# lijun9250lj/video-steganography-PCAMV

Measured on AMD Instinct MI355X. Metric: 1080p macroblocks/s (embed on), higher is better.
Workload: dtype u8

## Files before the change

### video-steganography-pcamv_amd/csrc/pcamv_prims_gpu.h

```cpp
#ifndef PCAMV_PRIMS_GPU_H
#define PCAMV_PRIMS_GPU_H
#include "pcamv_common.h"

__device__ __forceinline__ int pcamv_lane_id(void) { int l = (int)(threadIdx.x & 63); asm volatile("" : "+v"(l)); return l; }
#ifndef PCAMV_RD_LO
#define PCAMV_RD_LO 0
#endif
#define LANE() (PCAMV_RD_LO ? (int)(threadIdx.x & 63) : pcamv_lane_id())
__device__ __forceinline__ uint32_t clamp_u8(int v)
{
    asm volatile("" : "+v"(v));
    return (uint32_t)(v < 0 ? 0 : v > 255 ? 255 : v);
}
__device__ __forceinline__ uint32_t ld4u(const uint8_t *p) { uint32_t v; __builtin_memcpy(&v, p, 4); return v; }
__device__ __forceinline__ uint32_t lds4(const uint8_t *p) { return *(const uint32_t *)p; }
__device__ __forceinline__ void sts4(uint8_t *p, uint32_t v) { *(uint32_t *)p = v; }
__device__ __forceinline__ uint32_t avg4(uint32_t a, uint32_t b) { return __builtin_amdgcn_lerp(a, b, 0x01010101u); }
__device__ __forceinline__ int dpp_qp1(int v) { return __builtin_amdgcn_update_dpp(0, v, 0xB1, 0xf, 0xf, false); }
__device__ __forceinline__ int dpp_qp2(int v) { return __builtin_amdgcn_update_dpp(0, v, 0x4E, 0xf, 0xf, false); }
__device__ __forceinline__ int dpp_hmir(int v) { return __builtin_amdgcn_update_dpp(0, v, 0x141, 0xf, 0xf, false); }
__device__ __forceinline__ int dpp_mir(int v) { return __builtin_amdgcn_update_dpp(0, v, 0x140, 0xf, 0xf, false); }

__device__ __forceinline__ int group_sum(int v, int g)
{
    if (g >= 2) v += dpp_qp1(v);
    if (g >= 4) v += dpp_qp2(v);
    if (g >= 8) v += dpp_hmir(v);
    if (g >= 16) v += dpp_mir(v);
    return v;
}
__device__ __forceinline__ int wave_sum_all(int v)
{
    v = group_sum(v, 16);
    return __builtin_amdgcn_readlane(v, 0) + __builtin_amdgcn_readlane(v, 16) + __builtin_amdgcn_readlane(v, 32) + __builtin_amdgcn_readlane(v, 48);
}

__device__ __forceinline__ int hadamard4x4_abs(const uint32_t e[4], const uint32_t r[4])
{
    int t[4][4], s = 0;
#pragma unroll
    for (int y = 0; y < 4; y++) {
        int d0 = (int)(e[y] & 255) - (int)(r[y] & 255), d1 = (int)((e[y] >> 8) & 255) - (int)((r[y] >> 8) & 255);
        int d2 = (int)((e[y] >> 16) & 255) - (int)((r[y] >> 16) & 255), d3 = (int)(e[y] >> 24) - (int)(r[y] >> 24);
        int s01 = d0 + d1, d01 = d0 - d1, s23 = d2 + d3, d23 = d2 - d3;
        t[y][0] = s01 + s23; t[y][1] = d01 + d23; t[y][2] = s01 - s23; t[y][3] = d01 - d23;
    }
#pragma unroll
    for (int x = 0; x < 4; x++) {
        int s01 = t[0][x] + t[1][x], d01 = t[0][x] - t[1][x], s23 = t[2][x] + t[3][x], d23 = t[2][x] - t[3][x];
        s += iabs(s01 + s23) + iabs(d01 + d23) + iabs(s01 - s23) + iabs(d01 - d23);
    }
    return s;
}

__device__ __forceinline__ uint32_t chroma_row4(const FrameDev &F, int plane, int cx, int cy, int mvx, int mvy)
{
    int dx = mvx & 7, dy = mvy & 7;
    int cA = (8 - dx) * (8 - dy), cB = dx * (8 - dy), cC = (8 - dx) * dy, cD = dx * dy;
    const uint8_t *s = (plane ? F.chroma[1] : F.chroma[0]) + (ptrdiff_t)(cy + (mvy >> 3)) * F.cstride + cx + (mvx >> 3);
    uint32_t a0 = ld4u(s), a1 = s[4], b0 = ld4u(s + F.cstride), b1 = s[F.cstride + 4];
    uint32_t o = 0;
#pragma unroll
    for (int i = 0; i < 4; i++) {
        int p00 = (a0 >> (8 * i)) & 255, p01 = i < 3 ? (a0 >> (8 * i + 8)) & 255 : a1;
        int p10 = (b0 >> (8 * i)) & 255, p11 = i < 3 ? (b0 >> (8 * i + 8)) & 255 : b1;
        o |= (uint32_t)((cA * p00 + cB * p01 + cC * p10 + cD * p11 + 32) >> 6) << (8 * i);
    }
    return o;
}


__device__ __forceinline__ int rfl(int v) { return __builtin_amdgcn_readfirstlane(v); }
__device__ __forceinline__ int wave_min_i32(int v)
{
    v = imin(v, dpp_qp1(v)); v = imin(v, dpp_qp2(v)); v = imin(v, dpp_hmir(v)); v = imin(v, dpp_mir(v));
    return imin(imin(__builtin_amdgcn_readlane(v, 0), __builtin_amdgcn_readlane(v, 16)),
                imin(__builtin_amdgcn_readlane(v, 32), __builtin_amdgcn_readlane(v, 48)));
}

typedef const __attribute__((address_space(1))) uint8_t *gp8;
typedef const __attribute__((address_space(1))) int16_t *gp16;
typedef uint32_t __attribute__((aligned(1))) u32u;
typedef uint64_t __attribute__((aligned(1))) u64u;
typedef short v2s __attribute__((ext_vector_type(2)));
__device__ __forceinline__ uint32_t gld4(gp8 base, uint32_t off) { return *(const __attribute__((address_space(1))) u32u *)(base + off); }
__device__ __forceinline__ uint64_t gld8(gp8 base, uint32_t off) { return *(const __attribute__((address_space(1))) u64u *)(base + off); }
__device__ __forceinline__ int gld_cost(gp8 tab, uint32_t i) { return (int)*(const __attribute__((address_space(1))) int16_t *)(tab + (i << 1)); }
__device__ __forceinline__ int prim_mv_cost(const FrameDev &F, int d)
{
    const int i = rfl(d) + PCAMV_COST_MV_CENTRE;
    const __attribute__((address_space(4))) uint32_t *t = (const __attribute__((address_space(4))) uint32_t *)(F.cost_mv - PCAMV_COST_MV_CENTRE);
    const uint32_t w = t[i >> 1];
    return (int)(int16_t)(w >> (16 * (i & 1)));
}
__device__ __forceinline__ uint32_t mul24u(uint32_t a, uint32_t b) { return __umul24(a, b); }
__device__ __forceinline__ int mul24s(int a, int b) { return __mul24(a, b); }
__device__ __forceinline__ int mad24s(int a, int b, int c) { return __mul24(a, b) + c; }
__device__ __forceinline__ uint32_t lsw_x(uint32_t x, uint32_t lskip) { return mul24u(mul24u(x, 18725u) >> 19, lskip) + x; }
__device__ __forceinline__ v2s as_v2s(uint32_t v) { return __builtin_bit_cast(v2s, v); }
__device__ __forceinline__ uint32_t as_u32(v2s v) { return __builtin_bit_cast(uint32_t, v); }

__device__ __forceinline__ void pk_cols(const uint32_t r[4], uint32_t o[8])
{
#pragma unroll
    for (int x = 0; x < 4; x++) {
        const uint32_t sel = 0x0c040c00u + (uint32_t)x * 0x00010001u;
        o[x] = __builtin_amdgcn_perm(r[1], r[0], sel);
        o[4 + x] = __builtin_amdgcn_perm(r[3], r[2], sel);
    }
}
__device__ __forceinline__ int satd4x4_half(const uint32_t ec[8], const uint32_t r[4])
{
    uint32_t rc[8];
    pk_cols(r, rc);
    v2s t[8];
#pragma unroll
    for (int g = 0; g < 2; g++) {
        v2s d0 = as_v2s(ec[4 * g]) - as_v2s(rc[4 * g]), d1 = as_v2s(ec[4 * g + 1]) - as_v2s(rc[4 * g + 1]);
        v2s d2 = as_v2s(ec[4 * g + 2]) - as_v2s(rc[4 * g + 2]), d3 = as_v2s(ec[4 * g + 3]) - as_v2s(rc[4 * g + 3]);
        v2s s01 = d0 + d1, d01 = d0 - d1, s23 = d2 + d3, d23 = d2 - d3;
        t[4 * g] = s01 + s23; t[4 * g + 1] = d01 + d23; t[4 * g + 2] = s01 - s23; t[4 * g + 3] = d01 - d23;
    }
    v2s acc = {0, 0};
    const v2s z = {0, 0};
#pragma unroll
    for (int x = 0; x < 4; x++) {
        v2s S = t[x] + t[4 + x], D = t[x] - t[4 + x];
        v2s aS = __builtin_elementwise_max(S, z - S), aD = __builtin_elementwise_max(D, z - D);
        v2s U = as_v2s(__builtin_amdgcn_perm(as_u32(aD), as_u32(aS), 0x05040100u));
        v2s V = as_v2s(__builtin_amdgcn_perm(as_u32(aD), as_u32(aS), 0x07060302u));
        acc += __builtin_elementwise_max(U, V);
    }
    return (int)acc.x + (int)acc.y;
}

__device__ __forceinline__ void chroma_rows_load(gp8 cb, uint32_t cstride, uint32_t off, uint64_t row[5])
{
#pragma unroll
    for (int k = 0; k < 5; k++) row[k] = gld8(cb + (size_t)k * cstride, off);
}
__device__ __forceinline__ void chroma_block4_rows(const uint64_t row[5], int mvx, int mvy, uint32_t r[4])
{
    const int dx = mvx & 7, dy = mvy & 7;
    const uint32_t W = mul24u(8 - dx, 8 - dy) | mul24u(dx, 8 - dy) << 8 | mul24u(8 - dx, dy) << 16 | mul24u(dx, dy) << 24;
    uint32_t w[5][4];
#pragma unroll
    for (int k = 0; k < 5; k++) {
        const uint32_t lo = (uint32_t)row[k], hi = (uint32_t)(row[k] >> 32);
        w[k][0] = lo; w[k][1] = __builtin_amdgcn_alignbit(hi, lo, 8); w[k][2] = __builtin_amdgcn_alignbit(hi, lo, 16); w[k][3] = __builtin_amdgcn_alignbit(hi, lo, 24);
    }
#pragma unroll
    for (int k = 0; k < 4; k++) {
        uint32_t o = 0;
#pragma unroll
        for (int i = 0; i < 4; i++) {
            const uint32_t px = __builtin_amdgcn_perm(w[k + 1][i], w[k][i], 0x05040100u);
            o |= (__builtin_amdgcn_udot4(px, W, 32u, false) >> 6) << (8 * i);
        }
        r[k] = o;
    }
}
__device__ __forceinline__ void chroma_block4(gp8 cb, uint32_t cstride, uint32_t off, int mvx, int mvy, uint32_t r[4])
{
    uint64_t row[5];
    chroma_rows_load(cb, cstride, off, row);
    chroma_block4_rows(row, mvx, mvy, r);
}

__device__ __forceinline__ uint32_t wld4(const MBLocal *L, int b)
{
    const uint32_t *w = L->win + (b >> 2);
    return __builtin_amdgcn_alignbit(w[1], w[0], (uint32_t)(b & 3) * 8u);
}
__device__ __forceinline__ void prim_win_load(const FrameDev &F, MBLocal *L, int bmx, int bmy)
{
    PCAMV_WAVE_SYNC();
    const int lane = LANE();
    const int x0 = L->mb_x * 16 + PCAMV_PAD + ((bmx - 3) >> 2), y0 = L->mb_y * 16 + PCAMV_PAD + ((bmy - 3) >> 2);
    const int cx0 = L->mb_x * 8 + PCAMV_CPAD + ((bmx - 3) >> 3), cy0 = L->mb_y * 8 + PCAMV_CPAD + ((bmy - 3) >> 3);
    const gp8 lb = (gp8)F.luma_base, cb = (gp8)F.chroma_base[0];
    const uint32_t lskip = (uint32_t)F.lskip, psz = (uint32_t)F.plane_size, cstride = (uint32_t)F.cstride, cps = (uint32_t)F.cplane_size;
    for (int i = lane; i < 4 * WIN_LH * (WIN_LW / 4); i += 64) {
        const int pl = i / (WIN_LH * (WIN_LW / 4)), r = (i / (WIN_LW / 4)) % WIN_LH, c = i % (WIN_LW / 4);
        L->win[i] = gld4(lb, (uint32_t)pl * psz + (uint32_t)(y0 + r) * PCAMV_LROW + lsw_x((uint32_t)(x0 + 4 * c), lskip));
    }
    for (int i = lane; i < 2 * WIN_CH * (WIN_CW / 4); i += 64) {
        const int pl = i / (WIN_CH * (WIN_CW / 4)), r = (i / (WIN_CW / 4)) % WIN_CH, c = i % (WIN_CW / 4);
        L->win[4 * WIN_LP / 4 + i] = gld4(cb, (uint32_t)pl * cps + (uint32_t)(cy0 + r) * cstride + (uint32_t)(cx0 + 4 * c));
    }
    if (lane == 0) { L->win_x0 = x0; L->win_y0 = y0; L->win_cx0 = cx0; L->win_cy0 = cy0; }
    PCAMV_WAVE_SYNC();
}
__device__ __forceinline__ void chroma_block4_win(const MBLocal *L, int b, int mvx, int mvy, uint32_t r[4])
{
    const int dx = mvx & 7, dy = mvy & 7;
    const uint32_t W = mul24u(8 - dx, 8 - dy) | mul24u(dx, 8 - dy) << 8 | mul24u(8 - dx, dy) << 16 | mul24u(dx, dy) << 24;
    const uint32_t sh = (uint32_t)(b & 3) * 8u;
    uint32_t w[5][4];
#pragma unroll
    for (int k = 0; k < 5; k++) {
        const uint32_t *p = L->win + ((b + k * WIN_CW) >> 2);
        const uint32_t lo = __builtin_amdgcn_alignbit(p[1], p[0], sh), hi = __builtin_amdgcn_alignbit(p[2], p[1], sh);
        w[k][0] = lo; w[k][1] = __builtin_amdgcn_alignbit(hi, lo, 8); w[k][2] = __builtin_amdgcn_alignbit(hi, lo, 16); w[k][3] = __builtin_amdgcn_alignbit(hi, lo, 24);
    }
#pragma unroll
    for (int k = 0; k < 4; k++) {
        uint32_t o = 0;
#pragma unroll
        for (int i = 0; i < 4; i++) {
            const uint32_t px = __builtin_amdgcn_perm(w[k + 1][i], w[k][i], 0x05040100u);
            o |= (__builtin_amdgcn_udot4(px, W, 32u, false) >> 6) << (8 * i);
        }
        r[k] = o;
    }
}

struct EvalEnv { const int16_t *cost_mv; const uint8_t *luma_base, *chroma_base; long long plane_size, cplane_size; int lskip, cstride; int *trace; int trace_mb; };
__device__ __forceinline__ EvalRes eval_list_body(const EvalEnv &F, MBLocal *L, const uint8_t *enc, int ip_, int xoff_, int yoff_,
                                                  int n_, int flags_, int mvp0_, int mvp1_)
{
    const int ip = rfl(ip_), xoff = rfl(xoff_), yoff = rfl(yoff_), n = rfl(n_), flags = rfl(flags_), mvp0 = rfl(mvp0_), mvp1 = rfl(mvp1_);
    const int lane = LANE();
    const int lgn = lg_nblk_of(ip), lgw = lg_w4_of(ip), nblk = 1 << lgn;
    const int satd = flags & EV_SATD;
    const gp8 cost_tab = (gp8)(F.cost_mv - PCAMV_COST_MV_CENTRE);
    PCAMV_WAVE_SYNC();
    const unsigned long long t_ev = PROF_T();
    PROF_CNT(32, 1); PROF_CNT(33, n);
    int key_acc = 0x7fffffff;
    {
        const int slot = lane >> lgn, blk = lane & (nblk - 1);
        const int px = xoff + 4 * (blk & ((1 << lgw) - 1)), py = yoff + 4 * (blk >> lgw);
        uint32_t e[4], ec[8];
        const uint8_t *encl = (flags & EV_SRC4) ? enc + (slot & 3) * 384 : enc;
#pragma unroll
        for (int k = 0; k < 4; k++) e[k] = lds4(encl + (py + k) * 16 + px);
        if (satd) pk_cols(e, ec);
        const gp8 lb = (gp8)F.luma_base;
        const uint32_t stride = PCAMV_LROW, psz = (uint32_t)F.plane_size, lskip = (uint32_t)F.lskip;
        const gp8 lb1 = lb + stride, lb2 = lb1 + stride, lb3 = lb2 + stride;
        const uint32_t rowbase = (uint32_t)(L->mb_y * 16 + py + PCAMV_PAD) * stride, colbase = (uint32_t)(L->mb_x * 16 + px + PCAMV_PAD);
        const int cpp = 64 >> lgn;
        for (int p0 = 0; p0 < n; p0 += cpp) {
            const int c = p0 + slot;
            const uint32_t xy = L->cxy[c < n ? c : 0];
            const bool act = c < n && xy != CAND_NONE;
            const int mvx = act ? (int)(int16_t)(xy & 0xffffu) : 0, mvy = act ? (int)(int16_t)(xy >> 16) : 0;
            const uint32_t o = rowbase + (uint32_t)((mvy >> 2) * (int)stride) + lsw_x(colbase + (uint32_t)(mvx >> 2), lskip);
            int mvb0 = 0, mvb1 = 0;
            if (!(flags & EV_NOMV)) { mvb0 = gld_cost(cost_tab, (uint32_t)(mvx - mvp0 + PCAMV_COST_MV_CENTRE)); mvb1 = gld_cost(cost_tab, (uint32_t)(mvy - mvp1 + PCAMV_COST_MV_CENTRE)); }
            uint32_t r[4];
            if (flags & EV_WIN) {
                const int dx = mvx & 3, dy = mvy & 3;
                const int wb = (L->mb_y * 16 + py + PCAMV_PAD + (mvy >> 2) - L->win_y0) * WIN_LW + (L->mb_x * 16 + px + PCAMV_PAD + (mvx >> 2) - L->win_x0);
                const int ba = wb + ((dx != 0) + 2 * (dy == 2)) * WIN_LP + (dy == 3 ? WIN_LW : 0);
#pragma unroll
                for (int k = 0; k < 4; k++) r[k] = wld4(L, ba + k * WIN_LW);
                if ((dx | dy) & 1) {
                    const int bb = wb + (dy ? (2 + (dx == 2)) * WIN_LP : 0) + (dx == 3);
#pragma unroll
                    for (int k = 0; k < 4; k++) r[k] = avg4(r[k], wld4(L, bb + k * WIN_LW));
                }
            } else if (flags & EV_FPEL) {
                r[0] = gld4(lb, o); r[1] = gld4(lb1, o); r[2] = gld4(lb2, o); r[3] = gld4(lb3, o);
            } else {
                const int dx = mvx & 3, dy = mvy & 3;
                const uint32_t oa = o + (dx != 0 ? psz : 0u) + (dy == 2 ? 2u * psz : 0u) + (dy == 3 ? stride : 0u);
                r[0] = gld4(lb, oa); r[1] = gld4(lb1, oa); r[2] = gld4(lb2, oa); r[3] = gld4(lb3, oa);
                if ((dx | dy) & 1) {
                    const uint32_t ob = o + (dy ? (dx == 2 ? 3u * psz : 2u * psz) : 0u) + (dx == 3);
                    r[0] = avg4(r[0], gld4(lb, ob)); r[1] = avg4(r[1], gld4(lb1, ob));
                    r[2] = avg4(r[2], gld4(lb2, ob)); r[3] = avg4(r[3], gld4(lb3, ob));
                }
            }
            asm volatile("" : "+v"(mvb0), "+v"(mvb1), "+v"(r[0]), "+v"(r[1]), "+v"(r[2]), "+v"(r[3]));
            int v;
            if (satd) v = satd4x4_half(ec, r);
            else {
                uint32_t sa = 0;
#pragma unroll
                for (int k = 0; k < 4; k++) sa = __builtin_amdgcn_sad_u8(e[k], r[k], sa);
                v = (int)sa;
            }
            v = group_sum(v, nblk) + mvb0 + mvb1;
            if (blk == 0 && c < n) L->ccost[c] = act ? v : PCAMV_COST_MAX;
            if (blk == 0 && act) key_acc = imin(key_acc, (v << 6) | c);
        }
    }
    PCAMV_WAVE_SYNC();
    if ((flags & EV_CHROMA) && ip <= PIX_8x8) {
        const int lgnb = lgn - 2, nb = 1 << lgnb, lgcw = lgw - 1;
        const int slot = lane >> (lgnb + 1), plane = (lane >> lgnb) & 1, blk = lane & (nb - 1);
        const int px = (xoff >> 1) + 4 * (blk & ((1 << lgcw) - 1)), py = (yoff >> 1) + 4 * (blk >> lgcw);
        uint32_t e[4], ec[8];
        const uint8_t *encl = (flags & EV_SRC4) ? enc + (slot & 3) * 384 : enc;
#pragma unroll
        for (int k = 0; k < 4; k++) e[k] = lds4(encl + 256 + (py + k) * 16 + plane * 8 + px);
        if (satd) pk_cols(e, ec);
        const gp8 cb = (gp8)F.chroma_base;
        const uint32_t cstride = (uint32_t)F.cstride;
        const uint32_t rowbase = (plane ? (uint32_t)F.cplane_size : 0u) + mul24u((uint32_t)(L->mb_y * 8 + py + PCAMV_CPAD), cstride) + (uint32_t)(L->mb_x * 8 + px + PCAMV_CPAD);
        const int cpp = 64 >> (lgnb + 1);
        for (int p0 = 0; p0 < n; p0 += cpp) {
            const int c = p0 + slot;
            const uint32_t xy = L->cxy[c < n ? c : 0];
            const bool act = c < n && xy != CAND_NONE;
            const int mvx = act ? (int)(int16_t)(xy & 0xffffu) : 0, mvy = act ? (int)(int16_t)(xy >> 16) : 0;
            uint32_t r[4];
            if (flags & EV_WIN)
                chroma_block4_win(L, 4 * WIN_LP + plane * WIN_CP + (L->mb_y * 8 + py + PCAMV_CPAD + (mvy >> 3) - L->win_cy0) * WIN_CW
                                         + (L->mb_x * 8 + px + PCAMV_CPAD + (mvx >> 3) - L->win_cx0), mvx, mvy, r);
            else
                chroma_block4(cb, cstride, rowbase + (uint32_t)(mul24s(mvy >> 3, (int)cstride) + (mvx >> 3)), mvx, mvy, r);
            int v;
            if (satd) v = satd4x4_half(ec, r);
            else {
                uint32_t sa = 0;
#pragma unroll
                for (int k = 0; k < 4; k++) sa = __builtin_amdgcn_sad_u8(e[k], r[k], sa);
                v = (int)sa;
            }
            v = group_sum(v, nb);
            if (blk == 0 && act) {
                if (flags & EV_PROBE) L->ccost[64 * (1 + plane) + c] = v;
                else atomicAdd(&L->ccost[c], v);
            }
        }
    }
    PCAMV_WAVE_SYNC();
    int key = 0x7fffffff;
    if ((flags & EV_CHROMA) && ip <= PIX_8x8) { if (lane < n) { int cc = L->ccost[lane]; if (cc < PCAMV_COST_MAX) key = (cc << 6) | lane; } }
    else key = key_acc;
    key = wave_min_i32(key);
    EvalRes res;
    if (key == 0x7fffffff) { res.cost = PCAMV_COST_MAX; res.idx = -1; }
    else { res.cost = key >> 6; res.idx = key & 63; }
    PROF_ADD(38, t_ev);
#ifdef PCAMV_TRACE
    if (F.trace && L->mb_xy == F.trace_mb && lane == 0)
        for (int c = 0; c < n; c++) {
            if (L->cxy[c] == CAND_NONE) continue;
            int k = F.trace[0];
            if (k < 4000) { int *t = F.trace + 1 + 8 * k; t[0] = ip; t[1] = xoff; t[2] = yoff; t[3] = CAND_X(c); t[4] = CAND_Y(c); t[5] = flags | ((enc == L->recb || enc == L->recb0) ? 32 : 0); t[6] = L->ccost[c]; t[7] = c; F.trace[0] = k + 1; }
        }
#endif
    PCAMV_WAVE_SYNC();
    return res;
}

__device__ __forceinline__ EvalRes prim_eval_list(const FrameDev &F, MBLocal *L, const uint8_t *enc, int ip, int xoff, int yoff, int n, int flags, int mvp0, int mvp1)
{
    EvalEnv E;
    E.cost_mv = F.cost_mv; E.luma_base = F.luma_base; E.chroma_base = F.chroma_base[0]; E.plane_size = F.plane_size; E.cplane_size = F.cplane_size;
    E.lskip = F.lskip; E.cstride = F.cstride; E.trace = F.trace; E.trace_mb = F.trace_mb;
    return eval_list_body(E, L, enc, ip, xoff, yoff, n, flags, mvp0, mvp1);
}

__device__ __forceinline__ EvalRes prim_esa_window(const FrameDev &F, MBLocal *L, int ip_, int xoff_, int yoff_, int min_x_, int min_y_,
                                                   int width_, int nrows_, int mvp0_, int mvp1_)
{
    const int ip = rfl(ip_), xoff = rfl(xoff_), yoff = rfl(yoff_), min_x = rfl(min_x_), min_y = rfl(min_y_), width = rfl(width_), nrows = rfl(nrows_);
    const int mvp0 = rfl(mvp0_), mvp1 = rfl(mvp1_);
    const int lane = LANE();
    const int lgn = lg_nblk_of(ip), lgw = lg_w4_of(ip), nblk = 1 << lgn;
    const int slot = lane >> lgn, blk = lane & (nblk - 1), nslot = 64 >> lgn;
    const int px = xoff + 4 * (blk & ((1 << lgw) - 1)), py = yoff + 4 * (blk >> lgw);
    const gp8 cost_tab = (gp8)(F.cost_mv - PCAMV_COST_MV_CENTRE);
    PCAMV_WAVE_SYNC();
    uint32_t e[4];
#pragma unroll
    for (int k = 0; k < 4; k++) e[k] = lds4(L->fenc + (py + k) * 16 + px);
    const gp8 lb = (gp8)F.luma_raster;
    const uint32_t stride = (uint32_t)F.stride;
    const gp8 lb1 = lb + stride, lb2 = lb1 + stride, lb3 = lb2 + stride;
    const uint32_t rowbase = (uint32_t)(L->mb_y * 16 + py + PCAMV_PAD) * stride + (uint32_t)(L->mb_x * 16 + px + PCAMV_PAD);
    int best = 0x7fffffff;
    for (int r0 = 0; r0 < nrows; r0 += nslot) {
        const int ry = r0 + slot;
        const bool rowok = ry < nrows;
        const int my = min_y + (rowok ? ry : 0);
        const int ycost = gld_cost(cost_tab, (uint32_t)(my * 4 - mvp1 + PCAMV_COST_MV_CENTRE));
        const uint32_t orow = rowbase + (uint32_t)(my * (int)stride + min_x);
        for (int x0 = 0; x0 < width; x0 += 4) {
            const uint32_t o = orow + (uint32_t)x0;
            const uint64_t w0 = gld8(lb, o), w1 = gld8(lb1, o), w2 = gld8(lb2, o), w3 = gld8(lb3, o);
            uint32_t s[4];
#pragma unroll
            for (int j = 0; j < 4; j++) {
                const uint32_t sh = 8u * (uint32_t)j;
                uint32_t a = 0;
                a = __builtin_amdgcn_sad_u8(e[0], j ? __builtin_amdgcn_alignbit((uint32_t)(w0 >> 32), (uint32_t)w0, sh) : (uint32_t)w0, a);
                a = __builtin_amdgcn_sad_u8(e[1], j ? __builtin_amdgcn_alignbit((uint32_t)(w1 >> 32), (uint32_t)w1, sh) : (uint32_t)w1, a);
                a = __builtin_amdgcn_sad_u8(e[2], j ? __builtin_amdgcn_alignbit((uint32_t)(w2 >> 32), (uint32_t)w2, sh) : (uint32_t)w2, a);
                a = __builtin_amdgcn_sad_u8(e[3], j ? __builtin_amdgcn_alignbit((uint32_t)(w3 >> 32), (uint32_t)w3, sh) : (uint32_t)w3, a);
                s[j] = a;
            }
            int p01 = (int)(s[0] | s[1] << 16), p23 = (int)(s[2] | s[3] << 16);
            p01 = group_sum(p01, nblk); p23 = group_sum(p23, nblk);
            const int jn = nblk >= 4 ? 1 : 4;
            for (int jj = 0; jj < jn; jj++) {
                const int j = nblk >= 4 ? (blk & 3) : jj;
                const int sad = (j & 2 ? p23 : p01) >> (16 * (j & 1)) & 0xffff;
                const int mx = min_x + x0 + j;
                const int cost = sad + ycost + gld_cost(cost_tab, (uint32_t)(mx * 4 - mvp0 + PCAMV_COST_MV_CENTRE));
                const int key = (cost << 11) | (ry * width + x0 + j);
                if (rowok && x0 + j < width && key < best) best = key;
            }
        }
    }
    best = wave_min_i32(best);
    EvalRes res;
    if (best == 0x7fffffff) { res.cost = PCAMV_COST_MAX; res.idx = -1; }
    else { res.cost = best >> 11; res.idx = best & 2047; }
    PCAMV_WAVE_SYNC();
    return res;
}

__device__ __forceinline__ void prim_tesa_row(const FrameDev &F, MBLocal *L, int ip_, int xoff_, int yoff_, int min_x_, int my_, int width_, int mvp0_)
{
    const int ip = rfl(ip_), xoff = rfl(xoff_), yoff = rfl(yoff_), min_x = rfl(min_x_), my = rfl(my_), width = rfl(width_), mvp0 = rfl(mvp0_);
    const int lane = LANE();
    const int bw = pix_w_of(ip), bh = pix_h_of(ip), sub = ip <= PIX_8x8 ? 8 : 4;
    const gp8 cost_tab = (gp8)(F.cost_mv - PCAMV_COST_MV_CENTRE);
    const gp8 lb = (gp8)F.luma_raster;
    const uint32_t stride = (uint32_t)F.stride;
    PCAMV_WAVE_SYNC();
    if (lane < width) {
        const uint32_t base = (uint32_t)(L->mb_y * 16 + yoff + my + PCAMV_PAD) * stride + (uint32_t)(L->mb_x * 16 + xoff + min_x + lane + PCAMV_PAD);
        int sad = 0, rs0 = 0, rs1 = 0, rs2 = 0, rs3 = 0, es0 = 0, es1 = 0, es2 = 0, es3 = 0;
        for (int r = 0; r < bh; r++)
            for (int j = 0; j < bw; j += 4) {
                const uint32_t ref = gld4(lb, base + (uint32_t)r * stride + (uint32_t)j), e = lds4(L->fenc + (yoff + r) * 16 + xoff + j);
                sad = (int)__builtin_amdgcn_sad_u8(ref, e, (uint32_t)sad);
                const int rsum = (int)__builtin_amdgcn_sad_u8(ref, 0u, 0u), esum = (int)__builtin_amdgcn_sad_u8(e, 0u, 0u);
                const int k = (r >= sub ? 2 : 0) + (j >= sub ? 1 : 0);
                rs0 += k == 0 ? rsum : 0; rs1 += k == 1 ? rsum : 0; rs2 += k == 2 ? rsum : 0; rs3 += k == 3 ? rsum : 0;
                es0 += k == 0 ? esum : 0; es1 += k == 1 ? esum : 0; es2 += k == 2 ? esum : 0; es3 += k == 3 ? esum : 0;
            }
        const int ads = iabs(es0 - rs0) + iabs(es1 - rs1) + iabs(es2 - rs2) + iabs(es3 - rs3);
        L->ccost[lane] = sad + gld_cost(cost_tab, (uint32_t)(lane * 4 - mvp0 + PCAMV_COST_MV_CENTRE));
        L->ccost[64 + lane] = ads + gld_cost(cost_tab, (uint32_t)((min_x + lane) * 4 - mvp0 + PCAMV_COST_MV_CENTRE));
    }
    PCAMV_WAVE_SYNC();
}
__device__ __forceinline__ int prim_tesa_scan(MBLocal *L, int width_, int bsad_, int sad_thresh_, int ycost_, int ry_, int *n_)
{
    const int width = rfl(width_), bsad0 = rfl(bsad_), sad_thresh = rfl(sad_thresh_), ycost = rfl(ycost_), ry = rfl(ry_), n = rfl(*n_);
    const int lane = LANE();
    PCAMV_WAVE_SYNC();
    const bool look = lane < width && L->ccost[64 + lane] < bsad0 * 17 / 16;
    const int sad = lane < width ? L->ccost[lane] : 0;
    int incl = look ? sad : 0x7fffffff;
#pragma unroll
    for (int d = 1; d < 64; d <<= 1) { const int o = __shfl_up(incl, d); if (lane >= d) incl = imin(incl, o); }
    int before = __shfl_up(incl, 1);
    before = lane == 0 ? bsad0 : imin(bsad0, before);
    const bool keep = look && sad < (before * sad_thresh >> 3);
    const unsigned long long m = __ballot(keep);
    if (keep) *TESA_SLOT(L, n + __popcll(m & ((1ull << lane) - 1))) = TESA_PACK(sad + ycost, ry, lane);
    *n_ = n + __popcll(m);
    const int bsad = imin(bsad0, rfl(__shfl(incl, 63)));
    PCAMV_WAVE_SYNC();
    return bsad;
}
__device__ __forceinline__ int prim_tesa_select(MBLocal *L, int n_, int limit_, int bsad_, int sad_thresh_, int min_x_, int min_y_)
{
    int n = rfl(n_);
    const int limit = rfl(limit_), min_x = rfl(min_x_), min_y = rfl(min_y_);
    const int lane = LANE();
    PCAMV_WAVE_SYNC();
    if (n > limit * 2) {
        const int thr = rfl(bsad_) * (rfl(sad_thresh_) + 8) >> 4;
        int kept = 0;
        for (int b0 = 0; b0 < n; b0 += 64) {
            const uint32_t e = b0 + lane < n ? *TESA_SLOT(L, b0 + lane) : 0u;
            const bool keep = b0 + lane < n && TESA_SAD(e) <= thr;
            const unsigned long long m = __ballot(keep);
            PCAMV_WAVE_SYNC();
            if (keep) *TESA_SLOT(L, kept + __popcll(m & ((1ull << lane) - 1))) = e;
            kept += __popcll(m);
            PCAMV_WAVE_SYNC();
        }
        n = kept;
    }
    if (n > limit) {
        for (int i = 0; i < limit; i++) {
            int best = 0x7fffffff;
            for (int j = i + lane; j < n; j += 64) best = imin(best, (TESA_SAD(*TESA_SLOT(L, j)) << 11) | j);
            best = wave_min_i32(best);
            const int bj = best & 2047;
            if (lane == 0 && bj > i) { const uint32_t t = *TESA_SLOT(L, i); *TESA_SLOT(L, i) = *TESA_SLOT(L, bj); *TESA_SLOT(L, bj) = t; }
            PCAMV_WAVE_SYNC();
        }
        n = limit;
    }
    if (lane < n) { const uint32_t e = *TESA_SLOT(L, lane); L->cxy[lane] = CAND_PACK((min_x + (int)(e & 63)) * 4, (min_y + (int)(e >> 6 & 63)) * 4); }
    PCAMV_WAVE_SYNC();
    return n;
}

__device__ __forceinline__ int prim_chroma4x4_cost(const FrameDev &F, MBLocal *L, int i8, const int mv4x[4], const int mv4y[4], int satd)
{
    PCAMV_WAVE_SYNC();
    const int lane = LANE();
    int v = 0;
    if (lane < 2) {
        int ox = 4 * (i8 & 1), oy = 2 * (i8 & 2);
        uint32_t e[4], r[4];
#pragma unroll
        for (int k = 0; k < 4; k++) {
            uint32_t o = 0;
#pragma unroll
            for (int hlf = 0; hlf < 2; hlf++) {
                int q = (k >> 1) * 2 + hlf;
                uint32_t t = chroma_row4(F, lane, L->mb_x * 8 + ox + 2 * hlf, L->mb_y * 8 + oy + k, mv4x[q], mv4y[q]);
                o |= (t & 0xFFFFu) << (16 * hlf);
            }
            r[k] = o;
            e[k] = lds4(L->fenc + 256 + (oy + k) * 16 + lane * 8 + ox);
        }
        if (satd) v = hadamard4x4_abs(e, r) >> 1;
        else { uint32_t s = 0; for (int k = 0; k < 4; k++) s = __builtin_amdgcn_sad_u8(e[k], r[k], s); v = (int)s; }
    }
    v = group_sum(v, 2);
    return __builtin_amdgcn_readlane(v, 0);
}

__device__ __forceinline__ void prim_load_fenc(const FrameDev &F, MBLocal *L)
{
    const auto &D = FD(F);
    PCAMV_WAVE_SYNC();
    const int lane = LANE();
    { int row = lane >> 2, c4 = lane & 3;
      sts4(L->fenc + row * 16 + c4 * 4, *(const uint32_t *)(D.fenc[0] + (size_t)(L->mb_y * 16 + row) * D.w + L->mb_x * 16 + c4 * 4)); }
    if (lane < 32) {
        int plane = lane >> 4, row = (lane & 15) >> 1, c4 = lane & 1;
        sts4(L->fenc + 256 + row * 16 + plane * 8 + c4 * 4,
             *(const uint32_t *)((plane ? D.fenc[2] : D.fenc[1]) + (size_t)(L->mb_y * 8 + row) * (D.w >> 1) + L->mb_x * 8 + c4 * 4));
    }
    PCAMV_WAVE_SYNC();
}

__device__ __forceinline__ uint32_t luma_row4(const FrameDev &F, int gx, int gy, int mvx, int mvy)
{
    const gp8 lb = (gp8)F.luma_base;
    const uint32_t stride = PCAMV_LROW, psz = (uint32_t)F.plane_size;
    const uint32_t o = (uint32_t)(gy + PCAMV_PAD + (mvy >> 2)) * stride + lsw_x((uint32_t)(gx + PCAMV_PAD + (mvx >> 2)), (uint32_t)F.lskip);
    const int dx = mvx & 3, dy = mvy & 3;
    uint32_t r = gld4(lb, o + (dx != 0 ? psz : 0u) + (dy == 2 ? 2u * psz : 0u) + (dy == 3 ? stride : 0u));
    if ((dx | dy) & 1) r = avg4(r, gld4(lb, o + (dy ? (dx == 2 ? 3u * psz : 2u * psz) : 0u) + (dx == 3)));
    return r;
}
__device__ __forceinline__ uint32_t chroma_px2(const FrameDev &F, int plane, int cx, int cy, int mvx, int mvy)
{
    const gp8 cb = (gp8)F.chroma_base[0];
    const uint32_t cstride = (uint32_t)F.cstride;
    const uint32_t o = (plane ? (uint32_t)F.cplane_size : 0u) + mul24u((uint32_t)(cy + PCAMV_CPAD + (mvy >> 3)), cstride) + (uint32_t)(cx + PCAMV_CPAD + (mvx >> 3));
    const int dx = mvx & 7, dy = mvy & 7;
    const uint32_t W = mul24u(8 - dx, 8 - dy) | mul24u(dx, 8 - dy) << 8 | mul24u(8 - dx, dy) << 16 | mul24u(dx, dy) << 24;
    const uint32_t a = gld4(cb, o), b = gld4(cb + cstride, o);
    const uint32_t p0 = __builtin_amdgcn_udot4(__builtin_amdgcn_perm(b, a, 0x05040100u), W, 32u, false) >> 6;
    const uint32_t p1 = __builtin_amdgcn_udot4(__builtin_amdgcn_perm(b, a, 0x06050201u), W, 32u, false) >> 6;
    return p0 | p1 << 8;
}
__device__ __forceinline__ void prim_predict_mb(const FrameDev &F, MBLocal *L, int win)
{
    PCAMV_WAVE_SYNC();
    const int lane = LANE();
    { int row = lane >> 2, c4 = lane & 3, i8 = SCAN8_0 + c4 + 8 * (row >> 2);
      int mvx = clip3i(L->cmv[i8][0], L->mv_min[0], L->mv_max[0]), mvy = clip3i(L->cmv[i8][1], L->mv_min[1], L->mv_max[1]);
      uint32_t v;
      if (win) {
          const int dx = mvx & 3, dy = mvy & 3;
          const int wb = (L->mb_y * 16 + row + PCAMV_PAD + (mvy >> 2) - L->win_y0) * WIN_LW + (L->mb_x * 16 + 4 * c4 + PCAMV_PAD + (mvx >> 2) - L->win_x0);
          v = wld4(L, wb + ((dx != 0) + 2 * (dy == 2)) * WIN_LP + (dy == 3 ? WIN_LW : 0));
          if ((dx | dy) & 1) v = avg4(v, wld4(L, wb + (dy ? (2 + (dx == 2)) * WIN_LP : 0) + (dx == 3)));
      } else v = luma_row4(F, L->mb_x * 16 + 4 * c4, L->mb_y * 16 + row, mvx, mvy);
      sts4(L->pred + row * 16 + 4 * c4, v); }
    {
        int plane = lane >> 5, row = (lane & 31) >> 2, c2 = lane & 3;
        int i8 = SCAN8_0 + c2 + 8 * (row >> 1);
        int mvx = clip3i(L->cmv[i8][0], L->mv_min[0], L->mv_max[0]), mvy = clip3i(L->cmv[i8][1], L->mv_min[1], L->mv_max[1]);
        uint32_t t;
        if (win) {
            const int b = 4 * WIN_LP + plane * WIN_CP + (L->mb_y * 8 + row + PCAMV_CPAD + (mvy >> 3) - L->win_cy0) * WIN_CW + (L->mb_x * 8 + 2 * c2 + PCAMV_CPAD + (mvx >> 3) - L->win_cx0);
            const int dx = mvx & 7, dy = mvy & 7;
            const uint32_t W = mul24u(8 - dx, 8 - dy) | mul24u(dx, 8 - dy) << 8 | mul24u(8 - dx, dy) << 16 | mul24u(dx, dy) << 24;
            const uint32_t a = wld4(L, b), bb = wld4(L, b + WIN_CW);
            t = (__builtin_amdgcn_udot4(__builtin_amdgcn_perm(bb, a, 0x05040100u), W, 32u, false) >> 6)
              | (__builtin_amdgcn_udot4(__builtin_amdgcn_perm(bb, a, 0x06050201u), W, 32u, false) >> 6) << 8;
        } else t = chroma_px2(F, plane, L->mb_x * 8 + 2 * c2, L->mb_y * 8 + row, mvx, mvy);
        *(uint16_t *)(L->pred + 256 + row * 16 + plane * 8 + 2 * c2) = (uint16_t)t;
    }
    PCAMV_WAVE_SYNC();
}
__device__ __forceinline__ void prim_predict_16x16(const FrameDev &F, MBLocal *L, int mvx, int mvy, int which)
{
    PCAMV_WAVE_SYNC();
    const int lane = LANE();
    if (which != 2) { int row = lane >> 2, c4 = lane & 3; sts4(L->pred + row * 16 + 4 * c4, luma_row4(F, L->mb_x * 16 + 4 * c4, L->mb_y * 16 + row, mvx, mvy)); }
    if (which != 0) {
        int plane = lane >> 5, row = (lane & 31) >> 2, c2 = lane & 3;
        uint32_t t = chroma_px2(F, plane, L->mb_x * 8 + 2 * c2, L->mb_y * 8 + row, mvx, mvy);
        *(uint16_t *)(L->pred + 256 + row * 16 + plane * 8 + 2 * c2) = (uint16_t)t;
    }
    PCAMV_WAVE_SYNC();
// ... 439 lines not shown
```

### video-steganography-pcamv_amd/csrc/pcamv_rd.hip

```cpp
#include <hip/hip_runtime.h>
#include <stdint.h>
#include "pcamv_rd_select.h"
#ifndef PCAMV_RD_BUILD
#define PCAMV_RD_BUILD hi
#endif
#define RD_ID_(id) RD_##id
#define RD_ID(id) RD_ID_(id)
static constexpr int RD_BUILD = RD_ID(PCAMV_RD_BUILD);
#ifdef PCAMV_RD_OCC
static constexpr int RD_OCC = RD_BUILD == RD_hi ? PCAMV_RD_OCC : rd_build_defs[RD_BUILD].occ;
#else
static constexpr int RD_OCC = rd_build_defs[RD_BUILD].occ;
#endif
static constexpr int RD_VARIANT = rd_build_defs[RD_BUILD].variant;
static constexpr bool RD_ONE_WAVE = rd_build_defs[RD_BUILD].occ == 1;
#define PCAMV_RD_LO RD_ONE_WAVE
#define PCAMV_RESIDUAL_CALL 1
#include "pcamv_flow.hip.h"

static __global__ void __launch_bounds__(64, RD_OCC) k_analyse_flow_rd(const FrameDev *__restrict__ Fs, FlowDev fl)
{
    __shared__ MBLocal L;
    __shared__ Analysis A;
    flow_loop<0, RD_VARIANT>(Fs, fl, L, &A, nullptr);
}

template <> void pcamv_launch_flow_rd<RD_BUILD>(unsigned waves, hipStream_t st, const FrameDev *dF, const FlowDev &fl)
{
    hipLaunchKernelGGL(k_analyse_flow_rd, dim3(waves), dim3(64), 0, st, dF, fl);
}
template <> int pcamv_flow_rd_waves_per_cu<RD_BUILD>(void)
{
    int per_cu = 0;
    if (hipOccupancyMaxActiveBlocksPerMultiprocessor(&per_cu, k_analyse_flow_rd, 64, 0) != hipSuccess) return -1;
    return per_cu;
}
#ifdef PCAMV_PROF
template <> int pcamv_rd_prof_fetch<RD_BUILD>(unsigned long long *out, int reset)
{
    if (hipMemcpyFromSymbol(out, HIP_SYMBOL(pcamv_prof), sizeof(unsigned long long) * PCAMV_PROF_N) != hipSuccess) return -1;
    if (reset) { unsigned long long z[PCAMV_PROF_N] = {0}; if (hipMemcpyToSymbol(HIP_SYMBOL(pcamv_prof), z, sizeof(z)) != hipSuccess) return -1; }
    return 0;
}
#endif
```

### video-steganography-pcamv_amd/csrc/pcamv_tesa.hip

```cpp
#include <hip/hip_runtime.h>
#include <stdint.h>
#include "pcamv_flow.hip.h"

static __global__ void __launch_bounds__(64, PCAMV_FLOW_OCC) k_analyse_flow_tesa(const FrameDev *__restrict__ Fs, FlowDev fl)
{
    __shared__ MBLocal L;
    __shared__ Analysis A;
    flow_loop<0, V_TESA>(Fs, fl, L, &A, nullptr);
}

void pcamv_launch_flow_tesa(unsigned waves, hipStream_t st, const FrameDev *dF, const FlowDev &fl)
{
    hipLaunchKernelGGL(k_analyse_flow_tesa, dim3(waves), dim3(64), 0, st, dF, fl);
}
```

Measured before the change: 26.05 million.

## Compute 16x16 luma SATD via i8 MFMA Hadamard transform

Adds a matrix-core path for 16x16 luma SATD in candidate evaluation. It remaps lanes so each lane holds one row of a 4x4 block, then runs the Hadamard transform as an i8 MFMA against a constant ±1 operand, with a bias trick to keep signed differences. Absolute values are summed with sad_u16. This replaces the packed-v2s DPP butterfly SATD with the intent of offloading arithmetic to MFMA. It is disabled for the TESA variant, and it changes the lane mapping and candidates-per-pass, which adds MFMA latency and register pressure.

```diff
diff --git a/video-steganography-pcamv_amd/csrc/pcamv_prims_gpu.h b/video-steganography-pcamv_amd/csrc/pcamv_prims_gpu.h
--- a/video-steganography-pcamv_amd/csrc/pcamv_prims_gpu.h
+++ b/video-steganography-pcamv_amd/csrc/pcamv_prims_gpu.h
@@ -7,6 +7,9 @@
 #define PCAMV_RD_LO 0
 #endif
 #define LANE() (PCAMV_RD_LO ? (int)(threadIdx.x & 63) : pcamv_lane_id())
+#ifndef PCAMV_SATD_MAT
+#define PCAMV_SATD_MAT 1
+#endif
 __device__ __forceinline__ uint32_t clamp_u8(int v)
 {
     asm volatile("" : "+v"(v));
@@ -134,6 +137,29 @@
     return (int)acc.x + (int)acc.y;
 }
 
+typedef int v4i32 __attribute__((ext_vector_type(4)));
+#define SATD_BIAS 32768
+__device__ __forceinline__ long satd_mat_operand(int lane)
+{
+    const int n = lane & 15, g = lane >> 4, a = n >> 2, b = n & 3;
+    uint32_t pat = b == 0 ? 0x01010101u : b == 1 ? 0xff01ff01u : b == 2 ? 0xffff0101u : 0x01ffff01u;
+    if (__builtin_popcount(a & g) & 1) pat ^= 0xfefefefeu;
+    return (long)(((uint64_t)(pat ^ 0xfefefefeu) << 32) | pat);
+}
+__device__ __forceinline__ int satd16x16_rows_mat(const uint32_t e[4], const uint32_t r[4], long hb)
+{
+    const v4i32 bias = {SATD_BIAS, SATD_BIAS, SATD_BIAS, SATD_BIAS};
+    uint32_t s = 0;
+#pragma unroll
+    for (int j = 0; j < 4; j++) {
+        const long a = (long)(((uint64_t)(r[j] ^ 0x80808080u) << 32) | e[j]);
+        const v4i32 d = __builtin_amdgcn_mfma_i32_16x16x32_i8(a, hb, bias, 0, 0, 0);
+#pragma unroll
+        for (int i = 0; i < 4; i++) s = __builtin_amdgcn_sad_u16((uint32_t)d[i], (uint32_t)SATD_BIAS, s);
+    }
+    return group_sum((int)s, 16) >> 1;
+}
+
 __device__ __forceinline__ void chroma_rows_load(gp8 cb, uint32_t cstride, uint32_t off, uint64_t row[5])
 {
 #pragma unroll
@@ -215,6 +241,7 @@
     }
 }
 
+template <bool B> struct BoolC { static constexpr bool value = B; };
 struct EvalEnv { const int16_t *cost_mv; const uint8_t *luma_base, *chroma_base; long long plane_size, cplane_size; int lskip, cstride; int *trace; int trace_mb; };
 __device__ __forceinline__ EvalRes eval_list_body(const EvalEnv &F, MBLocal *L, const uint8_t *enc, int ip_, int xoff_, int yoff_,
                                                   int n_, int flags_, int mvp0_, int mvp1_)
@@ -228,20 +255,30 @@
     const unsigned long long t_ev = PROF_T();
     PROF_CNT(32, 1); PROF_CNT(33, n);
     int key_acc = 0x7fffffff;
-    {
-        const int slot = lane >> lgn, blk = lane & (nblk - 1);
-        const int px = xoff + 4 * (blk & ((1 << lgw) - 1)), py = yoff + 4 * (blk >> lgw);
+    auto luma = [&](auto mat) __attribute__((always_inline)) {
+        constexpr bool MAT = decltype(mat)::value;
+        constexpr int RS = MAT ? 4 : 1;
+        int slot, blk, px, py, cpp;
+        if (MAT) {
+            const int m = lane & 15, g = lane >> 4;
+            slot = m >> 2; blk = lane ^ mul24s(g, 20); px = xoff + 4 * (m & 3); py = yoff + g; cpp = 4;
+        } else {
+            slot = lane >> lgn; blk = lane & (nblk - 1); px = xoff + 4 * (blk & ((1 << lgw) - 1)); py = yoff + 4 * (blk >> lgw); cpp = 64 >> lgn;
+        }
         uint32_t e[4], ec[8];
         const uint8_t *encl = (flags & EV_SRC4) ? enc + (slot & 3) * 384 : enc;
 #pragma unroll
-        for (int k = 0; k < 4; k++) e[k] = lds4(encl + (py + k) * 16 + px);
-        if (satd) pk_cols(e, ec);
+        for (int k = 0; k < 4; k++) e[k] = lds4(encl + (py + k * RS) * 16 + px) ^ (MAT ? 0x80808080u : 0u);
+        if (!MAT && satd) pk_cols(e, ec);
+        const long hb = MAT ? satd_mat_operand(lane) : 0;
         const gp8 lb = (gp8)F.luma_base;
         const uint32_t stride = PCAMV_LROW, psz = (uint32_t)F.plane_size, lskip = (uint32_t)F.lskip;
-        const gp8 lb1 = lb + stride, lb2 = lb1 + stride, lb3 = lb2 + stride;
+        const gp8 lb1 = lb + RS * stride, lb2 = lb1 + RS * stride, lb3 = lb2 + RS * stride;
         const uint32_t rowbase = (uint32_t)(L->mb_y * 16 + py + PCAMV_PAD) * stride, colbase = (uint32_t)(L->mb_x * 16 + px + PCAMV_PAD);
-        const int cpp = 64 >> lgn;
         for (int p0 = 0; p0 < n; p0 += cpp) {
+            if (MAT || satd) PROF_CNT(39, 1);
+            if (MAT) PROF_CNT(31, 1);
+            if (MAT && (flags & EV_WIN)) PROF_CNT(23, 1);
             const int c = p0 + slot;
             const uint32_t xy = L->cxy[c < n ? c : 0];
             const bool act = c < n && xy != CAND_NONE;
@@ -255,11 +292,11 @@
                 const int wb = (L->mb_y * 16 + py + PCAMV_PAD + (mvy >> 2) - L->win_y0) * WIN_LW + (L->mb_x * 16 + px + PCAMV_PAD + (mvx >> 2) - L->win_x0);
                 const int ba = wb + ((dx != 0) + 2 * (dy == 2)) * WIN_LP + (dy == 3 ? WIN_LW : 0);
 #pragma unroll
-                for (int k = 0; k < 4; k++) r[k] = wld4(L, ba + k * WIN_LW);
+                for (int k = 0; k < 4; k++) r[k] = wld4(L, ba + k * RS * WIN_LW);
                 if ((dx | dy) & 1) {
                     const int bb = wb + (dy ? (2 + (dx == 2)) * WIN_LP : 0) + (dx == 3);
 #pragma unroll
-                    for (int k = 0; k < 4; k++) r[k] = avg4(r[k], wld4(L, bb + k * WIN_LW));
+                    for (int k = 0; k < 4; k++) r[k] = avg4(r[k], wld4(L, bb + k * RS * WIN_LW));
                 }
             } else if (flags & EV_FPEL) {
                 r[0] = gld4(lb, o); r[1] = gld4(lb1, o); r[2] = gld4(lb2, o); r[3] = gld4(lb3, o);
@@ -275,18 +312,20 @@
             }
             asm volatile("" : "+v"(mvb0), "+v"(mvb1), "+v"(r[0]), "+v"(r[1]), "+v"(r[2]), "+v"(r[3]));
             int v;
-            if (satd) v = satd4x4_half(ec, r);
+            if (MAT) v = satd16x16_rows_mat(e, r, hb);
+            else if (satd) v = satd4x4_half(ec, r);
             else {
                 uint32_t sa = 0;
 #pragma unroll
                 for (int k = 0; k < 4; k++) sa = __builtin_amdgcn_sad_u8(e[k], r[k], sa);
                 v = (int)sa;
             }
-            v = group_sum(v, nblk) + mvb0 + mvb1;
+            v = (MAT ? v : group_sum(v, nblk)) + mvb0 + mvb1;
             if (blk == 0 && c < n) L->ccost[c] = act ? v : PCAMV_COST_MAX;
             if (blk == 0 && act) key_acc = imin(key_acc, (v << 6) | c);
         }
-    }
+    };
+    if (PCAMV_SATD_MAT && satd && ip == PIX_16x16) luma(BoolC<true>()); else luma(BoolC<false>());
     PCAMV_WAVE_SYNC();
     if ((flags & EV_CHROMA) && ip <= PIX_8x8) {
         const int lgnb = lgn - 2, nb = 1 << lgnb, lgcw = lgw - 1;
@@ -302,6 +341,7 @@
         const uint32_t rowbase = (plane ? (uint32_t)F.cplane_size : 0u) + mul24u((uint32_t)(L->mb_y * 8 + py + PCAMV_CPAD), cstride) + (uint32_t)(L->mb_x * 8 + px + PCAMV_CPAD);
         const int cpp = 64 >> (lgnb + 1);
         for (int p0 = 0; p0 < n; p0 += cpp) {
+            if (satd) PROF_CNT(47, 1);
             const int c = p0 + slot;
             const uint32_t xy = L->cxy[c < n ? c : 0];
             const bool act = c < n && xy != CAND_NONE;
diff --git a/video-steganography-pcamv_amd/csrc/pcamv_rd.hip b/video-steganography-pcamv_amd/csrc/pcamv_rd.hip
--- a/video-steganography-pcamv_amd/csrc/pcamv_rd.hip
+++ b/video-steganography-pcamv_amd/csrc/pcamv_rd.hip
@@ -15,6 +15,7 @@
 static constexpr int RD_VARIANT = rd_build_defs[RD_BUILD].variant;
 static constexpr bool RD_ONE_WAVE = rd_build_defs[RD_BUILD].occ == 1;
 #define PCAMV_RD_LO RD_ONE_WAVE
+#define PCAMV_SATD_MAT (!(RD_VARIANT & V_TESA))
 #define PCAMV_RESIDUAL_CALL 1
 #include "pcamv_flow.hip.h"
 
diff --git a/video-steganography-pcamv_amd/csrc/pcamv_tesa.hip b/video-steganography-pcamv_amd/csrc/pcamv_tesa.hip
--- a/video-steganography-pcamv_amd/csrc/pcamv_tesa.hip
+++ b/video-steganography-pcamv_amd/csrc/pcamv_tesa.hip
@@ -1,5 +1,6 @@
 #include <hip/hip_runtime.h>
 #include <stdint.h>
+#define PCAMV_SATD_MAT 0
 #include "pcamv_flow.hip.h"
 
 static __global__ void __launch_bounds__(64, PCAMV_FLOW_OCC) k_analyse_flow_tesa(const FrameDev *__restrict__ Fs, FlowDev fl)
```

Result: faster. 26.45 million (median of 6 runs) (+1.5%).
